# Sartor02/libMultiRobotPlanning

Measured on AMD Instinct MI355X. Metric: low_level_node_expansions_per_sec, higher is better.
Workload: dtype int32

## Files before the change

### libmultirobotplanning_amd/csrc/ll_compact.h

```cpp
#pragma once
#include <stddef.h>
#include <stdint.h>

namespace mrp {
namespace ct {

using namespace wv;

#ifndef WV_HAS_UNMASKED_GLOADS
WV_FN V gLoadU16(const uint16_t* base, V idx) { return gLoadU16m(base, idx, bsplat(true)); }
WV_FN V gLoad32(const uint32_t* base, V idx) { return gLoad32m(base, idx, bsplat(true)); }
#endif

constexpr uint32_t kRowBytes = 128;
constexpr uint32_t oCtl = 0;
constexpr uint32_t oJob = 256;
constexpr uint32_t oRes = 384;
constexpr uint32_t oOpen = 448;
constexpr uint32_t kFront = 0xFFFFFFFFu;
template <uint32_t GROUPS, uint32_t FH_BITS, uint32_t F_BITS, uint32_t L_BITS, bool LONGT = false>
struct TierCfg {
  static constexpr bool kLongT = LONGT;
  static constexpr uint32_t kGroups = GROUPS;
  static constexpr uint32_t kCap = 256u * GROUPS - 1u;
// ... 27 lines not shown
  static constexpr uint32_t pathsOff(bool bg) { return obstOff(bg) + kRowBytes; }
  static constexpr uint32_t windowBytes(bool bg) { return pathsOff(bg); }
  static_assert(kFhShift + FH_BITS == 32u, "an entry is 32 bits");
  static_assert(!LONGT || L_BITS == 6u, "h <= 62 on a 32 x 32 map");
  static constexpr uint32_t kBuildRows = LONGT ? kRows : (2u * kHeapBytes >= kRows * kRowBytes ? kRows : kRows / 2u);
  static constexpr uint32_t kStageRows = (2u * kHeapBytes + kAuxBytes) / 1024u >= 8u ? 8u : (2u * kHeapBytes + kAuxBytes) / 1024u;
  static_assert(2u * kHeapBytes >= kBuildRows * kRowBytes && kRows % kBuildRows == 0u, "room for a chunk of bitmap rows");
  static_assert(kStageRows >= 4u, "room for the goal branch's rows");
  static_assert(!LONGT || kAuxBytes >= kBitsBytes, "LONGT builds a chunk of bitmap rows in the walk queue's area");
  static_assert(oFocal % 16 == 0 && oAux % 16 == 0 && oBits % 16 == 0 && oObst % 16 == 0 && oPaths % 16 == 0, "16-byte aligned areas");
  static_assert((kHeapClamp & 1u) == 1u && 4u * (kHeapClamp + 3u) <= kHeapBytes, "clamped child pair stays inside the heap area");
  static_assert((kAuxClamp & 1u) == 1u && 4u * (kAuxClamp + 3u) <= kAuxBytes, "clamped child pair stays inside the walk queue");
  static_assert(256u * GROUPS <= kAuxIdxMask + 1u && 10u + F_BITS + L_BITS + kAuxShift <= 32u, "walk-queue entry: key above index");
  static_assert(kMaxT + 1u + 62u <= kFMax - 3u, "f = g + h (h <= 62 on a 32 x 32 map) fits its field");
};
#ifndef MRP_CT_NARROW_GROUPS
#define MRP_CT_NARROW_GROUPS 4
#endif
typedef TierCfg<MRP_CT_NARROW_GROUPS, 9, 7, 6> Narrow;
#ifndef MRP_CT_WIDE_GROUPS
#define MRP_CT_WIDE_GROUPS 12
#endif
typedef TierCfg<MRP_CT_WIDE_GROUPS, 6, 10, 6, true> Wide;
constexpr uint32_t kGroups = Narrow::kGroups, kCap = Narrow::kCap, kHeapBytes = Narrow::kHeapBytes, kAuxBytes = Narrow::kAuxBytes;
constexpr uint32_t kRows = Narrow::kRows;
constexpr uint32_t oFocal = Narrow::oFocal, oAux = Narrow::oAux, oBits = Narrow::oBits, oObst = Narrow::oObst, oPaths = Narrow::oPaths;
constexpr uint32_t kLdsBytes = oPaths;
constexpr uint32_t obstOff(bool bg) { return Narrow::obstOff(bg); }
constexpr uint32_t pathsOff(bool bg) { return Narrow::pathsOff(bg); }
constexpr uint32_t windowBytes(bool bg) { return Narrow::windowBytes(bg); }
constexpr uint32_t kBitsBytes = Narrow::kBitsBytes, kParentBytes = Narrow::kParentBytes;
constexpr uint32_t kMO = Narrow::kMO, kMF = Narrow::kMF, kEmpty = Narrow::kEmpty, kMaxT = Narrow::kMaxT;
constexpr uint32_t kHeapClamp = Narrow::kHeapClamp;
static_assert(oOpen % 16 == 0, "LDS areas are 16-byte aligned");

enum : int32_t { C_OK = 0, C_NO_SOLUTION = 1, C_CAP_EXP = 2, C_OVERFLOW = -1 };

struct CJob {
  uint32_t dimx, dimy, sx, sy, gx, gy;
  int32_t lastGoal;
  float w;
  uint32_t nVc, nEc;
  uint32_t obstWords;
  uint32_t nAgentsPad, tPad;
  uint32_t maxExp;
  uint32_t openCap, maxT;
  uint32_t taNoGoal;
  uint32_t rows;
  uint64_t vc;
  uint64_t ec;
  uint64_t obst;
  uint64_t pathsG;
  uint64_t parentTab;
  uint64_t outPath;
  uint64_t bitsG;
};
static_assert(sizeof(CJob) <= oRes - oJob && sizeof(CJob) % 4 == 0, "CJob fits its block of the window");
struct CRes {
  int32_t status, cost, fmin, nStates;
  uint32_t expanded, nodes;
};
#ifdef MRP_CT_PROF
#define MRP_CT_PROF_DECL uint32_t prof_[8] = {0, 0, 0, 0, 0, 0, 0, 0}; uint64_t profT_ = wv::clock64()
#define MRP_CT_PROF_MARK(k) do { const uint64_t n_ = wv::clock64(); prof_[k] += (uint32_t)(n_ - profT_); profT_ = n_; } while (0)
#define MRP_CT_PROF_ADD(k, v) prof_[k] += (v)
#define MRP_CT_PROF_STORE(lds) do { for (uint32_t q_ = 0; q_ < 8; ++q_) ldsStoreS(lds, oRes + 32u + 4u * q_, prof_[q_]); } while (0)
#elif defined(MRP_CT_ASM_MARKS)
#define MRP_CT_PROF_DECL do { } while (0)
#define MRP_CT_PROF_MARK(k) asm volatile("; PHASE " #k ::: "memory")
#define MRP_CT_PROF_ADD(k, v) do { } while (0)
#define MRP_CT_PROF_STORE(lds) do { } while (0)
#else
#define MRP_CT_PROF_DECL do { } while (0)
#define MRP_CT_PROF_MARK(k) do { } while (0)
#define MRP_CT_PROF_ADD(k, v) do { } while (0)
#define MRP_CT_PROF_STORE(lds) do { } while (0)
#endif
static_assert(sizeof(CRes) <= 32 && oRes + 64 <= oOpen, "CRes fits its block of the window");

#ifndef MRP_CT_COUNT
#define MRP_CT_COUNT(k, v) do { } while (0)
#endif
#ifndef MRP_CT_COUNT_SLOTS
#define MRP_CT_COUNT_SLOTS 7
#endif
#define MRP_CT_COUNTX(k, v) do { if ((k) < MRP_CT_COUNT_SLOTS) MRP_CT_COUNT(k, v); } while (0)

#define MRP_CT_JOB_U32(lds, field) ldsLoadS(lds, oJob + (uint32_t)offsetof(CJob, field))
template <class T>
WV_FN T* jobPtr(Lds lds, uint32_t off) {
  const uint64_t lo = ldsLoadS(lds, oJob + off), hi = ldsLoadS(lds, oJob + off + 4u);
  return (T*)(uintptr_t)(lo | (hi << 32));
}
#define MRP_CT_JOB_PTR(T, lds, field) jobPtr<T>(lds, (uint32_t)offsetof(CJob, field))

WV_FN uint32_t popc64(uint64_t v) { return (uint32_t)__builtin_popcountll(v); }
WV_FN uint32_t ctz64(uint64_t v) { return (uint32_t)__builtin_ctzll(v); }
WV_FN uint32_t ctz32(uint32_t v) { return (uint32_t)__builtin_ctz(v); }
WV_FN uint32_t lg2(uint32_t v) { return 31u - (uint32_t)__builtin_clz(v); }
WV_FN uint32_t lo32(uint64_t v) { return (uint32_t)v; }
WV_FN uint32_t hi32(uint64_t v) { return (uint32_t)(v >> 32); }

#ifndef WV_HAS_CTZ
WV_FN V ctz(V v) { return splat(31u) - clz(v & (splat(0u) - v)); }
#endif

#ifdef MRP_CT_PLAIN_EXPANSION
#ifndef MRP_CT_SCALAR_PUSHES
// ... 290 lines not shown
  const V dx = sel(lane == 1u, splat(0xFFFFFFFFu), sel(lane == 2u, splat(1u), sel(lane < 5u, splat(0u), splat(0x4000u))));
  const V dy = sel(lane == 3u, splat(1u), sel(lane == 4u, splat(0xFFFFFFFFu), splat(0u)));
#ifndef MRP_CT_PLAIN_EXPANSION
  const bool grid = EPS && nAgentsPad != 0u && nAgentsPad <= 16u;
#else
  const bool grid = false;
#endif
  const V agent0 = grid ? Rw.l4 : lane;
  const B in0 = agent0 < nAgentsPad, in1 = (lane + 64u) < nAgentsPad;
  const V col0 = sel(in0, agent0, splat(nAgentsPad ? nAgentsPad - 1u : 0u));
  const V col1 = sel(in1, lane + 64u, splat(nAgentsPad ? nAgentsPad - 1u : 0u));
  const V gridD = perRow(Rw, 0xFFFFFFFFu, 1u, 256u, 0xFFFFFF00u);
  const V gridSh = ((lane - 1u) & 3u) << 4;
  const V gridWait = sel(lane == 0u, splat(0xFFFFFFFFu), splat(0u));
  const uint32_t tPad = EPS ? MRP_CT_JOB_U32(lds, tPad) : 0u;
  const uint16_t* pathsG = PLDS ? nullptr : MRP_CT_JOB_PTR(const uint16_t, lds, pathsG);
  const int32_t lastGoal = (int32_t)MRP_CT_JOB_U32(lds, lastGoal);
  const float wBound = uintAsFloat(MRP_CT_JOB_U32(lds, w));
  const uint32_t maxExp = MRP_CT_JOB_U32(lds, maxExp), openCap = MRP_CT_JOB_U32(lds, openCap), maxT = MRP_CT_JOB_U32(lds, maxT);
  uint8_t* parentTab = MRP_CT_JOB_PTR(uint8_t, lds, parentTab);
  const uint32_t goalCell = gx | (gy << 5);
  int32_t bestF;
  V tops;
  {
    const uint32_t sx = MRP_CT_JOB_U32(lds, sx), sy = MRP_CT_JOB_U32(lds, sy);
    const uint32_t h0 = (sx > gx ? sx - gx : gx - sx) + (sy > gy ? sy - gy : gy - sy);
    bestF = (int32_t)h0;
    const uint32_t e0 = (kFhMax << kFhShift) | ((kFMax - h0) << kFShift) | ((C::kLongT ? 63u - h0 : 0u) << 10) | (sx | (sy << 5));
    ldsStoreS(lds, oOpen + 4u, e0);
    if (EPS) ldsStoreS(lds, oFocal + 4u, e0);
    tops = splat(e0);
  }
  sync();
  MRP_CT_PROF_MARK(0);

  for (;;) {
    if (nOpen == 0u) {
      status = C_NO_SOLUTION;
      break;
    }
#ifdef MRP_CT_LOAD_TOPS
    tops = ldsLoad32(lds, hb);
#elif defined(MRP_CT_CHECK_TOPS)
    {
      const V seen = ldsLoad32(lds, hb);
      MRP_CT_COUNTX(8, 1u);
      MRP_CT_COUNTX(9, (readlane(seen, 0) != readlane(tops, 0) || (EPS && readlane(seen, 32) != readlane(tops, 32))) ? 1u : 0u);
    }
#endif
    const uint32_t topO = readlane(tops, 0);
    uint32_t curE = EPS ? readlane(tops, 32) : topO;
    if (EPS) {
      const int32_t fTop = (int32_t)(kFMax - ((topO >> kFShift) & kFMax));
      const int32_t oldBest = bestF;
      bestF = fTop;
      if (fTop > oldBest) {
        MRP_CT_PROF_MARK(0);
        const float lo = fmulRn((float)oldBest, wBound), hi = fmulRn((float)fTop, wBound);
        bool bandEmpty = false;
#ifndef MRP_CT_FORCE_WALK
        {
          const int32_t fA = (int32_t)lo + 1, fBraw = (int32_t)hi;
          const int32_t fB = fBraw > (int32_t)kFMax - 1 ? (int32_t)kFMax - 1 : fBraw;
          bandEmpty = true;
          if (fB >= fA) {
            const V base = splat(kFMax - (uint32_t)fB), span = splat((uint32_t)(fB - fA));
            for (uint32_t g = 0; g < kGroups && g * 256u <= nOpen; ++g) {
// ... 76 lines not shown
          }
        }
        for (uint32_t b = 0; b <= 4u * npqHigh; b += 1024u) {
          const V4 none{splat(kEmpty), splat(kEmpty), splat(kEmpty), splat(kEmpty)};
          const V4 head{sel(lane == 0u, splat(kFront), splat(kEmpty)), splat(kEmpty), splat(kEmpty), splat(kEmpty)};
          ldsStore128m(lds, splat(oAux + b) + lane * 16u, b == 0u ? head : none, (lane * 16u + b) < kAuxBytes);
        }
        if (status == C_OVERFLOW) break;
        curE = ldsLoadS(lds, oFocal + 4u);
#ifndef MRP_CT_LOAD_TOPS
        tops = sel(S.isB, splat(curE), tops);
#endif
        }
        MRP_CT_PROF_MARK(1);
      }
    }
    const uint32_t cell = curE & 1023u, curFh = kFhMax - (curE >> kFhShift);
    const uint32_t t = C::kLongT ? (kFMax - ((curE >> kFShift) & kFMax)) - (63u - ((curE >> 10) & 63u)) : (curE >> 10) & kGMax;
    const uint32_t x = cell & 31u, y = cell >> 5;
    const bool isGoal = cell == goalCell && (int32_t)t > lastGoal;
    if (!isGoal) {
      if (nOpen + 5u > openCap || t > maxT || (EPS && !C::kExactFhCheck && curFh + 2u * nAgentsPad > kFhMax)) {
        status = C_OVERFLOW;
        cost = nOpen + 5u > openCap ? 1 : t > maxT ? 2 : 3;
        break;
      }
    }
    expansions += 1u;
    if (expansions > maxExp) {
      status = C_CAP_EXP;
      break;
    }
    if (isGoal) {
      status = C_OK;
      cost = (int32_t)t;
      fmin = (int32_t)(kFMax - (((EPS ? topO : curE) >> kFShift) & kFMax));
      nStates = (int32_t)t + 1;
      uint16_t* outPath = MRP_CT_JOB_PTR(uint16_t, lds, outPath);
      sync();
      uint32_t c = cell;
      const uint32_t* tab32 = (const uint32_t*)parentTab;
      constexpr int32_t kStage = BG ? (int32_t)C::kStageRows : 8;
      for (int32_t k0 = (int32_t)t; k0 >= 1; k0 -= kStage) {
        V rowW[kStage][4];
        for (int32_t r = 0; r < kStage; ++r)
          for (uint32_t q = 0; q < 4; ++q)
            rowW[r][q] = (k0 - r >= 1) ? gLoad32Coherent(tab32, splat((uint32_t)(k0 - r) * 256u + q * 64u) + lane) : splat(0u);
        for (int32_t r = 0; r < kStage; ++r)
          for (uint32_t q = 0; q < 4; ++q) ldsStore32(lds, splat(oBuild + (uint32_t)r * 1024u + q * 256u) + lane * 4u, rowW[r][q]);
        sync();
        for (int32_t r = 0; r < kStage && k0 - r >= 1; ++r) {
          const uint32_t k = (uint32_t)(k0 - r);
          gStoreU16m(outPath, splat(k), splat((c & 31u) | ((c >> 5) << 8)), lane == 0u);
          const uint32_t a = first(ldsLoadU8(lds, splat(oBuild + (uint32_t)r * 1024u + c)));
          c = a == 1u ? c + 1u : a == 2u ? c - 1u : a == 3u ? c - 32u : a == 4u ? c + 32u : c;
        }
        sync();
      }
      gStoreU16m(outPath, splat(0u), splat((c & 31u) | ((c >> 5) << 8)), lane == 0u);
      break;
    }

    MRP_CT_PROF_MARK(0);
    const uint32_t t1 = t + 1u;
    if (C::kLongT && t1 >= rowsReady) moreRows();
    const V nx = splat(x) + dx, ny = splat(y) + dy;
    const B inb = (nx < dimx) & (ny < dimy);
    const V ncell = (nx & 31u) | ((ny & 31u) << 5);
    const V wordAddr = splat(oBits + t1 * kRowBytes) + ((ny & 31u) << 2);
    const V wordIdx = splat(t1 * (kRowBytes / 4u)) + (ny & 31u);
    const V word = BG ? gLoad32(bitsG, wordIdx) : ldsLoad32(lds, wordAddr);
    V a0 = splat(0xFFFFu), b0 = splat(0xFFFFu), a1 = splat(0xFFFFu), b1 = splat(0xFFFFu);
    if (EPS && nAgentsPad) {
      const uint32_t ra = t < tPad ? t : tPad - 1u;
      const uint32_t rb = t1 < tPad ? t1 : tPad - 1u;
      if (PLDS) {
        a0 = sel(in0, ldsLoadU16(lds, splat(oPathsX + ra * nAgentsPad * 2u) + col0 * 2u), splat(0xFFFFu));
        b0 = sel(in0, ldsLoadU16(lds, splat(oPathsX + rb * nAgentsPad * 2u) + col0 * 2u), splat(0xFFFFu));
        if (nAgentsPad > 64u) {
          a1 = sel(in1, ldsLoadU16(lds, splat(oPathsX + ra * nAgentsPad * 2u) + col1 * 2u), splat(0xFFFFu));
          b1 = sel(in1, ldsLoadU16(lds, splat(oPathsX + rb * nAgentsPad * 2u) + col1 * 2u), splat(0xFFFFu));
        }
      } else {
        a0 = gLoadU16(pathsG, splat(ra * nAgentsPad) + col0);
        b0 = gLoadU16(pathsG, splat(rb * nAgentsPad) + col0);
        if (nAgentsPad > 64u) {
          a1 = gLoadU16(pathsG, splat(ra * nAgentsPad) + col1);
          b1 = gLoadU16(pathsG, splat(rb * nAgentsPad) + col1);
        }
      }
    }

// ... 420 lines not shown
```

### libmultirobotplanning_amd/csrc/ll_jobs.h

```cpp
#ifndef MRP_LL_JOBS_H
#define MRP_LL_JOBS_H

namespace mrp {

__host__ __device__ inline uint32_t ldsBytes(uint32_t pathBytes, bool bg) { return ct::windowBytes(bg) + pathBytes; }

DEVI uint32_t storeLoad(const uint16_t* p) {
#ifdef MRP_LL_STORE_ACQUIRE_FENCE
  return *p;
#else
  return __hip_atomic_load(p, __ATOMIC_RELAXED, __HIP_MEMORY_SCOPE_AGENT);
#endif
}

DEVI uint32_t hostLoad32(const uint32_t* p) { return __hip_atomic_load(p, __ATOMIC_RELAXED, __HIP_MEMORY_SCOPE_SYSTEM); }
DEVI void hostStore32(uint32_t* p, uint32_t v) { __hip_atomic_store(p, v, __ATOMIC_RELAXED, __HIP_MEMORY_SCOPE_SYSTEM); }

DEVI void stageConstraints(const uint32_t* consHost, uint32_t vcOff, uint32_t nVc, uint32_t nEc, uint32_t* consLocal,
                           const uint32_t*& vc, const uint32_t*& ec) {
  const uint32_t* src = consHost + vcOff;
  const uint32_t nWords = nVc + nEc;
  if (nWords <= kConsLocalWords) {
    for (uint32_t i = threadIdx.x; i < nWords; i += 64) consLocal[i] = hostLoad32(src + i);
    vc = consLocal;
  } else {
    __builtin_amdgcn_fence(__ATOMIC_ACQUIRE, "");
    vc = src;
  }
  ec = vc + nVc;
}

__device__ __attribute__((noinline)) bool stageConstraintSet(const DevJob* job, const uint32_t* cons, uint32_t* store, uint32_t stride,
                                                             uint32_t slots, uint32_t* consLocal) {
  const uint32_t nVc = rfl(job->n_vc), nEc = rfl(job->n_ec), dimx = rfl(job->dimx), dimy = rfl(job->dimy);
  const uint32_t baseP1 = rfl(job->pad_[0]), baseCounts = rfl(job->pad_[1]), resP1 = rfl(job->pad_[2]);
  const uint32_t* added = cons + rfl(job->vc_off);
  stride = rfl(stride); slots = rfl(slots);
  const uint32_t bVc = baseP1 ? (baseCounts & 0xFFFFu) : 0u, bEc = baseP1 ? (baseCounts >> 16) : 0u;
  const uint32_t nWords = nVc + nEc;
  if (store == nullptr || baseP1 > slots || resP1 > slots || bVc > nVc || bEc > nEc || nVc > kConsLocalWords ||
      nEc > kConsLocalWords || nWords > kConsLocalWords || nWords > stride)
    return false;
  const uint32_t aVc = nVc - bVc;
  const uint32_t cells = dimx * dimy;
  const uint32_t* base = store + (size_t)(baseP1 ? baseP1 - 1u : 0u) * stride;
  uint32_t* out = store + (size_t)(resP1 ? resP1 - 1u : 0u) * stride;
  for (uint32_t i = threadIdx.x; i < nWords; i += 64) {
    uint32_t w;
    if (i < nVc) {
// ... 197 lines not shown
  }
  return true;
}

template <bool EPS, bool BG, int TIERS>
DEVI bool compactAttempt(const LaunchParams& P, const DevJob& J, uint8_t* smem, uint8_t* arenaSlot, const Ctx& c, DevResult& res,
                         uint16_t* outPath, SState& s, int& rc) {
  typedef typename std::conditional<TIERS == kTiersHeavy, ct::Wide, ct::Narrow>::type Geo;
  uint32_t geoRows = Geo::kRows;
  if (TIERS == kTiersHeavy) {
    const uint64_t room = slot::nodeBytes(P.arena_nodes) / (1024u + ct::kRowBytes);
    geoRows = (uint32_t)(room < P.arena_rows ? room : P.arena_rows) & ~63u;
  }
  const bool compactOk = !(TIERS == kTiersAll && (J.ctx_flags & kCtxHeavy) != 0) && P.lds_nodes != 0 && c.dimx <= 32u &&
                         c.dimy <= 32u && c.nAgentsPad <= 128u && c.nEc <= 64u && geoRows >= 64u &&
                         compactFits<Geo>(P.arena_nodes, geoRows, BG);
  bool done = false;
  if (compactOk) {
    ct::CJob cj = baseCJob<Geo>(P, J, arenaSlot, outPath, geoRows);
    cj.obstWords = c.wpr;
    cj.sx = c.sx; cj.sy = c.sy; cj.gx = c.gx; cj.gy = c.gy;
    cj.lastGoal = c.lastGoal;
    cj.nVc = c.nVc; cj.nEc = c.nEc;
    cj.nAgentsPad = EPS ? c.nAgentsPad : 0u; cj.tPad = c.tPad;
    cj.rows = geoRows;
    if (TIERS == kTiersHeavy) {
      cj.openCap = Geo::kCap;
      cj.maxT = Geo::kMaxT < geoRows - 2u ? Geo::kMaxT : geoRows - 2u;
    }
    cj.vc = (uint64_t)c.vc; cj.ec = (uint64_t)c.ec;
    cj.pathsG = (uint64_t)c.paths;
    putCJob(smem, cj);
    const bool tableInLds = !EPS || c.nAgentsPad == 0u || c.pathsLds != nullptr;
#ifndef MRP_LL_TRACE
    const uint64_t tl0 = __builtin_amdgcn_s_memrealtime();
#endif
    int32_t crc;
    if constexpr (TIERS == kTiersHeavy)
      crc = ct::compactSearch<EPS, false, BG, ct::Wide>((wv::Lds)smem);
    else
      crc = tableInLds ? ct::compactSearch<EPS, true, BG>((wv::Lds)smem) : ct::compactSearch<EPS, false, BG>((wv::Lds)smem);
    const ct::CRes cr = getCRes(smem);
#ifndef MRP_LL_TRACE
    res.prof[TIERS == kTiersHeavy ? 2 : 0] = (uint32_t)(__builtin_amdgcn_s_memrealtime() - tl0);
    res.prof[TIERS == kTiersHeavy ? 3 : 1] = cr.expanded;
#endif
#ifdef MRP_CT_PROF
    {
      auto r32 = (__attribute__((address_space(3))) const uint32_t*)((wv::Lds)smem + ct::oRes + 32u);
      for (uint32_t q = 0; q < 8; ++q) res.prof[q] = rfl(r32[q]);
    }
#endif
    if (crc != ct::C_OVERFLOW) {
      rc = crc;
      res.cost = cr.cost; res.fmin = cr.fmin; res.n_states = cr.nStates;
      s.expansions = cr.expanded; s.nNodes = cr.nodes;
      done = true;
      if (TIERS == kTiersHeavy) res.tier = 2;
    } else {
#ifndef MRP_LL_TRACE
      res.prof[6] = cr.expanded;
      res.prof[7] = 1;
#endif
    }
  }
  return done;
}

template <bool EPS, bool BG, int TIERS>
DEVI int arenaAttempt(const LaunchParams& P, uint8_t* smem, uint8_t* arenaSlot, const Ctx& c, DevResult& res, uint16_t* outPath,
                      SState& s) {
  typedef typename std::conditional<TIERS == kTiersHeavy, ct::Wide, ct::Narrow>::type Geo;
  int rc;
  const Mem<TierHbm> g = cutArena(P, arenaSlot);
  Mem<TierHyb> gh = viewAs<TierHyb>(g);
  {
    const uint32_t area = Geo::windowBytes(BG) - ct::oOpen;
#ifdef MRP_LL_TOPS_EQUAL
    const uint32_t perO = (area / 3u) & ~15u, perF = perO, perA = perO;
#else
    const uint32_t perO = (area / 2u) & ~15u, perF = (area * 5u / 16u) & ~15u, perA = (area - perO - perF) & ~15u;
#endif
    auto tops = [&](uint32_t per) {
      uint32_t n = per >= 32u ? ((per - 8u) / 8u) : 0u;
      if (n > 4095u) n = 4095u;
      n = n ? ((n - 1u) | 1u) : 0u;
      return P.lds_nodes == 0 ? 0u : n;
    };
    auto l8 = (__attribute__((address_space(3))) uint8_t*)smem + ct::oOpen;
    gh.open = HybPtr{(__attribute__((address_space(3))) uint64_t*)(l8 + 8), (uint64_t*)g.open, tops(perO)};
    gh.focal = HybPtr{(__attribute__((address_space(3))) uint64_t*)(l8 + perO + 8), (uint64_t*)g.focal, tops(perF)};
    gh.aux = HybPtr{(__attribute__((address_space(3))) uint64_t*)(l8 + perO + perF + 8), (uint64_t*)g.aux, tops(perA)};
  }
  const bool xyEntries = P.arena_nodes <= 65536u;
  Mem<TierHybXy> ghx = viewAs<TierHybXy>(gh);
  res.tier = 1;
  __syncthreads();
  if (xyEntries)
    initSearch<TierHybXy, EPS>(ghx, s, c);
  else
    initSearch<TierHyb, EPS>(gh, s, c);
  __syncthreads();
#ifndef MRP_LL_TRACE
  const uint64_t th0 = __builtin_amdgcn_s_memrealtime();
#endif
  if (xyEntries)
    rc = runSearch<TierHybXy, EPS>(ghx, s, c, res, outPath);
  else
    rc = runSearch<TierHyb, EPS>(gh, s, c, res, outPath);
#ifndef MRP_LL_TRACE
  if (TIERS != kTiersHeavy) {
    res.prof[2] = (uint32_t)(__builtin_amdgcn_s_memrealtime() - th0);
    res.prof[3] = (uint32_t)s.expansions;
  }
#endif
  return rc;
}

template <bool EPS, bool BG, int TIERS>
DEVI bool runJob(const LaunchParams& P, const DevJob& J, uint8_t* smem, uint8_t* arenaSlot, DevResult& res,
                 uint16_t* outPath) {
  typedef typename std::conditional<TIERS == kTiersHeavy, ct::Wide, ct::Narrow>::type Geo;
  if (TIERS == kTiersFront && frontHandsOver(P, J)) return true;
  Ctx c;
  fillCtx(c, J, P.maps, P.debug);
  uint32_t* consLocal = slot::consCopy(arenaSlot, P.arena_scratch_off, P.out_stride);
  if ((J.pad_[0] | J.pad_[2]) != 0u) {
    c.vc = consLocal;
    c.ec = consLocal + c.nVc;
  } else {
    stageConstraints(P.cons, J.vc_off, c.nVc, c.nEc, consLocal, c.vc, c.ec);
  }
  if (!stageFocalTable<TIERS>(P, J, smem + Geo::windowBytes(BG), slot::pathsCopy(arenaSlot, P.arena_scratch_off, P.out_stride), c)) {
    res.status = ST_BAD; res.expanded = 0; res.nodes_created = 0;
    return false;
  }
  __syncthreads();
  SState s;
  int rc = ST_BAD;
  res.tier = 0;
  if (!compactAttempt<EPS, BG, TIERS>(P, J, smem, arenaSlot, c, res, outPath, s, rc)) {
    if constexpr (TIERS == kTiersFront)
      return true;
    else
      rc = arenaAttempt<EPS, BG, TIERS>(P, smem, arenaSlot, c, res, outPath, s);
  }
  if (rc == RUN_MIGRATE_NODES) rc = ST_CAP_NODES;
  if (rc == RUN_MIGRATE_ROWS) rc = ST_CAP_HORIZON;
  res.status = rc;
  res.expanded = s.expansions;
  res.nodes_created = s.nNodes;
  return false;
}

template <class SidFn>
DEVI void publishPath(const LaunchParams& P, const uint16_t* outPath, uint32_t len, uint32_t* hostDst, SidFn sidOf) {
  const uint32_t lane = threadIdx.x;
  const uint32_t* src = (const uint32_t*)outPath;
  for (uint32_t i = lane; i < (len + 1u) / 2u; i += 64) hostStore32(hostDst + i, src[i]);
  const uint32_t sid = sidOf();
  if (sid < P.path_store_slots && len < P.path_store_stride) {
    uint16_t* slot = P.path_store + (size_t)sid * P.path_store_stride;
    for (uint32_t i = lane; i < len; i += 64) __hip_atomic_store(slot + 1 + i, outPath[i], __ATOMIC_RELAXED, __HIP_MEMORY_SCOPE_AGENT);
    __hip_atomic_store(slot, (uint16_t)len, __ATOMIC_RELAXED, __HIP_MEMORY_SCOPE_AGENT);
  }
}

template <bool HOSTLOADS>
DEVI void beginJob(const DevJob* jobSrc, DevJob& jobS, DevResult& res, uint32_t tier) {
  const uint32_t lane = threadIdx.x;
  const uint32_t* src = (const uint32_t*)jobSrc;
  __syncthreads();
  if (lane < sizeof(DevJob) / 4) ((uint32_t*)&jobS)[lane] = HOSTLOADS ? hostLoad32(src + lane) : src[lane];
  __syncthreads();
  res.status = ST_BAD; res.cost = 0; res.fmin = 0; res.n_states = 0; res.expanded = 0; res.nodes_created = 0;
  res.tier = tier;
  for (int q = 0; q < 8; ++q) res.prof[q] = 0;
}
DEVI void endJob(const DevResult& res, DevResult& resS, DevResult* resDst) {
  __syncthreads();
  resS = res;
  __syncthreads();
  if (threadIdx.x < sizeof(DevResult) / 4) hostStore32((uint32_t*)resDst + threadIdx.x, ((const uint32_t*)&resS)[threadIdx.x]);
}

DEVI void runChain(const LaunchParams& P, const DevJob& J, uint8_t* smem, uint8_t* arenaSlot, DevResult& res,
                   uint16_t* outPath, uint16_t* hostOut) {
  constexpr bool BG = true;
  const uint32_t lane = threadIdx.x;
  const uint32_t n = J.n_ctx, first = J.t_pad, npad = J.n_agents_pad;
  const uint32_t end = J.reserved > first && J.reserved < n ? J.reserved : n;
  res.tier = 0; res.n_states = 0; res.expanded = 0;
  if (P.lds_nodes == 0 || J.dimx > 32u || J.dimy > 32u || n > kChainMaxAgents || first >= n || npad < n || npad > 128u ||
      (npad & 1u) || kChainRows * npad * 2u > (P.lds_paths_bytes != 0u ? P.lds_paths_bytes : P.arena_paths_bytes) ||
      !compactFits<ct::Narrow>(P.arena_nodes, 0, BG) ||
      (uint64_t)n * kChainEntryWords * 2u + (uint64_t)n * 64u > (uint64_t)P.out_host_stride) {
    res.status = ST_BAD;
    return;
  }
  const uint32_t* who = P.cons + J.vc_off;
  const uint32_t* ids = who + n;
  const bool tabInLds = P.lds_paths_bytes != 0u;
  uint16_t* table = (uint16_t*)(tabInLds ? smem + ldsBytes(0, BG) : slot::pathsCopy(arenaSlot, P.arena_scratch_off, P.out_stride));
  for (uint32_t i = lane; i < kChainRows * npad / 2u; i += 64) ((uint32_t*)table)[i] = 0xFFFFFFFFu;
  __syncthreads();
  for (uint32_t a = 0; a < first; ++a) {
    const uint32_t id = rfl(hostLoad32(ids + a));
    if (id >= P.path_store_slots) continue;
    const uint16_t* slot = P.path_store + (size_t)id * P.path_store_stride;
    uint32_t len = rfl(storeLoad(slot));
    if (len > P.path_store_stride - 1) len = P.path_store_stride - 1;
    if (len == 0) continue;
    table[lane * npad + a] = (uint16_t)storeLoad(slot + 1 + (lane < len ? lane : len - 1));
  }
  __syncthreads();
  int64_t budget = J.max_expansions;
  uint32_t* hostW = (uint32_t*)hostOut;
  uint32_t pathOff = n * kChainEntryWords;
  uint32_t done = 0, maxLen = 0;
  bool allOk = true;
  int64_t total = 0;
  for (uint32_t a = first; a < end; ++a) {
    asm volatile("" : "+s"(hostW), "+s"(outPath));
    const uint32_t sg = rfl(hostLoad32(who + a));
    ct::CJob cj = baseCJob(P, J, arenaSlot, outPath);
    cj.sx = sg & 0xFFu; cj.sy = (sg >> 8) & 0xFFu; cj.gx = (sg >> 16) & 0xFFu; cj.gy = sg >> 24;
    cj.lastGoal = -1;
    cj.nVc = 0; cj.nEc = 0;
    cj.nAgentsPad = npad; cj.tPad = kChainRows;
    cj.maxExp = clampMaxExp(budget);
    cj.vc = 0; cj.ec = 0;
    cj.pathsG = tabInLds ? 0ull : (uint64_t)table;
    __syncthreads();
    putCJob(smem, cj);
#ifndef MRP_LL_TRACE
    const uint64_t tl0 = __builtin_amdgcn_s_memrealtime();
#endif
    const int32_t crc = tabInLds ? ct::compactSearch<true, true, BG>((wv::Lds)smem) : ct::compactSearch<true, false, BG>((wv::Lds)smem);
    const ct::CRes cr = getCRes(smem);
    const int32_t cost = cr.cost, fmin = cr.fmin, nStates = cr.nStates;
    const uint32_t expanded = cr.expanded;
#ifndef MRP_LL_TRACE
    res.prof[0] += (uint32_t)(__builtin_amdgcn_s_memrealtime() - tl0);
    res.prof[1] += expanded;
#endif
    if (crc == ct::C_OVERFLOW) {
#ifndef MRP_LL_TRACE
      res.prof[6] += expanded;
      res.prof[7] += 1;
#endif
      allOk = false;
      break;
    }
    {
      uint32_t v = 0;
      v = lane == 0 ? (uint32_t)crc : lane == 1 ? (uint32_t)cost : lane == 2 ? (uint32_t)fmin
          : lane == 3 ? (crc == ct::C_OK ? (uint32_t)nStates : 0u) : lane == 4 ? expanded : lane == 5 ? pathOff : 0u;
      if (lane < kChainEntryWords) hostStore32(hostW + (size_t)done * kChainEntryWords + lane, v);
    }
    done += 1;
    total += expanded;
    if (crc != ct::C_OK) {
      allOk = false;
      break;
    }
    const uint32_t len = (uint32_t)nStates;
    maxLen = len > maxLen ? len : maxLen;
    {
      publishPath(P, outPath, len, hostW + pathOff, [&] { return rfl(hostLoad32(ids + a)); });
      pathOff += (len + 1u) / 2u;
      uint32_t rowLen = npad;
      asm volatile("" : "+s"(rowLen));
      table[lane * rowLen + a] = outPath[lane < len ? lane : len - 1];
    }
    if (budget >= 0) budget = budget > (int64_t)expanded ? budget - (int64_t)expanded : 0;
  }
  __syncthreads();
  res.status = ST_OK;
  res.n_states = (int32_t)done;
  res.expanded = total;
  res.cost = -1;
  res.fmin = -1;
  if (first == 0 && end == n && done == n && allOk && maxLen >= 1u && maxLen <= kChainRows) {
    const uint32_t T = maxLen - 1u;
    uint32_t cnt = 0, key = 0x7FFFFFFFu;
    auto pairsOf = [&](const uint16_t* tab, uint32_t rowC, uint32_t rowN, uint32_t t, bool inT) {
      uint32_t bestV = 0xFFFFu, bestE = 0xFFFFu;
      for (uint32_t i = 0; i + 1u < n; ++i) {
        const uint32_t ci = tab[rowC + i], ni = tab[rowN + i];
        for (uint32_t j = i + 1u; j < n; ++j) {
          const uint32_t cj = tab[rowC + j], nj = tab[rowN + j];
          const bool v = inT && ci == cj, e = inT && ci == nj && ni == cj;
          cnt += (v ? 1u : 0u) + (e ? 1u : 0u);
          if (v && bestV == 0xFFFFu) bestV = (i << 8) | j;
          if (e && bestE == 0xFFFFu) bestE = (i << 8) | j;
        }
      }
      const uint32_t k = bestV != 0xFFFFu ? (t << 24) | bestV : bestE != 0xFFFFu ? (t << 24) | (1u << 16) | bestE : 0x7FFFFFFFu;
      key = k < key ? k : key;
    };
    if (tabInLds) {
      pairsOf(table, lane * npad, (lane + 1u < kChainRows ? lane + 1u : kChainRows - 1u) * npad, lane, lane < T);
    } else {
      uint16_t* stage = (uint16_t*)(smem + ct::oOpen);
      static_assert(2u * ct::kHeapBytes >= 32u * kChainMaxAgents * 2u, "room for 32 rows of the widest table");
      const uint32_t rowsFit = 2u * ct::kHeapBytes / (npad * 2u) < kChainRows ? 2u * ct::kHeapBytes / (npad * 2u) : kChainRows;
      for (uint32_t r0 = 0; r0 < T; r0 += rowsFit - 1u) {
        const uint32_t nRows = kChainRows - r0 < rowsFit ? kChainRows - r0 : rowsFit;
        __syncthreads();
        for (uint32_t i = lane; i < nRows * npad / 2u; i += 64) ((uint32_t*)stage)[i] = ((const uint32_t*)table)[r0 * npad / 2u + i];
        __syncthreads();
        const bool inT = lane + 1u < nRows && r0 + lane < T;
        const uint32_t row = inT ? lane : 0u;
        pairsOf(stage, row * npad, (row + 1u) * npad, r0 + lane, inT);
      }
    }
#pragma unroll
    for (uint32_t off = 32; off >= 1; off >>= 1) {
      cnt += (uint32_t)__shfl_xor((int)cnt, (int)off, 64);
      const uint32_t other = (uint32_t)__shfl_xor((int)key, (int)off, 64);
      key = other < key ? other : key;
    }
    res.cost = (int32_t)rfl(cnt);
    res.fmin = rfl(key) == 0x7FFFFFFFu ? -1 : (int32_t)rfl(key);
  }
}

}

#endif
```

### libmultirobotplanning_amd/csrc/ll_kernel.hip

```cpp
#include <hip/hip_runtime.h>
#include <stdint.h>

#include <mutex>
#include <type_traits>

#include "ll_device.h"
#include "ll_slot.h"
#include "ll_launch.h"
#include "wave_dev.h"
#include "ll_compact.h"

#include "ll_arena_heap.h"
#include "ll_arena_search.h"
#include "ll_jobs.h"
#include "ll_ta.h"
#include "ll_ta_root.h"
#include "ll_ta_eps_root.h"
#include "ll_sipp.h"
#include "ll_node_scan.h"

namespace mrp {

constexpr uint32_t kScanJobOff = ct::oCtl + sizeof(DevJob) + sizeof(DevResult), kScanOutOff = kScanJobOff + sizeof(ns::NsJob);
constexpr uint32_t kScanBaseOff = ct::oCtl + sizeof(DevJob);
// ... 63 lines not shown
                     uint8_t* arenaSlot, DevJob& jobS, DevResult& resS) {
  static_assert(TIERS == kTiersAll || KIND == 1, "front / heavy workgroups exist for the A*-epsilon sessions");
  const DevJob& J = jobS;
  DevResult res;
  beginJob<true>(jobSrc, jobS, res, 0);
  PROF_T0();
#ifndef MRP_LL_TRACE
  const uint64_t tj0 = __builtin_amdgcn_s_memrealtime();
#endif
  uint16_t* outPath = slot::outPath(arenaSlot, P.arena_scratch_off, P.out_stride);
  uint32_t algo = rfl(J.algo);
  bool handOver = false;
  if ((rfl(J.pad_[0]) | rfl(J.pad_[2])) != 0u && !(TIERS == kTiersFront && frontHandsOver(P, J))) {
    if (algo > 1u || (rfl(J.ctx_flags) & kCtxChain) ||
        !stageConstraintSet(&jobS, P.cons, P.cons_store, P.cons_store_stride, P.cons_store_slots,
                            slot::consCopy(arenaSlot, P.arena_scratch_off, P.out_stride)))
      algo = 0xFFFFFFFFu;
  }
  if constexpr (KIND == 0) {
    if (algo == 1)
      runJob<true, false, kTiersAll>(P, J, smem, arenaSlot, res, outPath);
    else if (algo == 3)
      runJobTA(P, J, smem, arenaSlot, res, outPath);
    else if (algo == 4) {
      const uint64_t th0 = __builtin_amdgcn_s_memrealtime();
      runJobTaEps<false>(&jobS, &resS, arenaSlot, P.maps, P.cons, P.paths, P.arena_scratch_off, P.out_stride, P.arena_nodes,
                  P.arena_rows, P.arena_row_words, P.arena_paths_bytes, P.path_store, P.path_store_stride, P.path_store_slots);
      __syncthreads();
      res.status = rfli(resS.status); res.cost = rfli(resS.cost); res.fmin = rfli(resS.fmin);
      res.n_states = rfli(resS.n_states);
      res.expanded = (int64_t)rfl64((uint64_t)resS.expanded);
      res.nodes_created = rfl(resS.nodes_created);
      res.tier = rfl(resS.tier);
      res.prof[2] = (uint32_t)(__builtin_amdgcn_s_memrealtime() - th0);
      res.prof[3] = (uint32_t)res.expanded;
    } else if (algo == 0)
      runJob<false, false, kTiersAll>(P, J, smem, arenaSlot, res, outPath);
  } else if constexpr (KIND == 1) {
    if (algo == 1) {
      if (rfl(J.ctx_flags) & kCtxChain) {
        if constexpr (TIERS != kTiersHeavy) runChain(P, J, smem, arenaSlot, res, outPath, pathDst);
      } else {
        handOver = runJob<true, true, TIERS>(P, J, smem, arenaSlot, res, outPath);
      }
    }
  } else {
    if (algo == 0) runJob<false, false, kTiersAll>(P, J, smem, arenaSlot, res, outPath);
    if (algo == 3) runJobTA(P, J, smem, arenaSlot, res, outPath);
  }
  if (TIERS == kTiersFront && handOver) return true;
  if constexpr (KIND != 2) {
    if (rfl(J.ctx_flags) & kCtxScan)
      scanNode<KIND == 1, TIERS>(P, J, smem, arenaSlot, (int32_t)rfl((uint32_t)res.status), rfl((uint32_t)res.n_states), outPath, pathDst);
  }
  PROF_ADD(res, 5);
#if !defined(MRP_LL_TRACE) && !defined(MRP_CT_PROF)
  res.prof[4] = (uint32_t)(__builtin_amdgcn_s_memrealtime() - tj0);
  res.prof[5] = 1;
#endif
  DBG(P, 2, res.status + 100);
  endJob(res, resS, resDst);
  if (res.status == ST_OK && !(KIND == 1 && (rfl(J.ctx_flags) & kCtxChain)))
    publishPath(P, outPath, (uint32_t)res.n_states, (uint32_t*)pathDst, [&] { return rfl(J.store_out_id); });
  return false;
}

static_assert(sizeof(DevJob) + sizeof(DevResult) <= ct::oJob, "control block of the window");
#define MRP_LL_WINDOW_BLOCKS(smem, jobS, resS)                                                        \
  if ((uint32_t)(uintptr_t)(__attribute__((address_space(3))) uint8_t*)smem != 0u) __builtin_trap(); \
  DevJob& jobS = *(DevJob*)(smem + ct::oCtl);                                                         \
  DevResult& resS = *(DevResult*)(smem + ct::oCtl + sizeof(DevJob))
#define MRP_LL_WINDOW_KERNEL(NAME, ...)                                                  \
  extern "C" __global__ void __launch_bounds__(64) NAME(LaunchParams Parg) {             \
    extern __shared__ __attribute__((aligned(16))) uint8_t smem[];                       \
    MRP_LL_WINDOW_BLOCKS(smem, jobS, resS);                                              \
    const LaunchParams& P = Parg;                                                        \
    __VA_ARGS__(P, smem, jobS, resS);                                                    \
  }
template <int KIND>
DEVI void batchLoop(const LaunchParams& P, uint8_t* smem, DevJob& jobS, DevResult& resS) {
  const uint32_t lane = threadIdx.x;
  uint8_t* arenaSlot = P.arena + (size_t)blockIdx.x * P.arena_stride;
  DBG(P, 0, 1);
  for (;;) {
    uint32_t j = atomicAdd(P.queue_head, lane == 0 ? 1u : 0u);
    j = rfl(j) - P.queue_base;
    DBG(P, 1, j + 1);
    if (j >= P.n_jobs) break;
    processJob<KIND>(P, P.jobs + j, P.results + j, P.out_paths + (size_t)j * P.out_host_stride, smem, arenaSlot, jobS, resS);
// ... 317 lines not shown
```

Before: 1.487 billion.

## Keep goal path in lanes and stage chain pairs to skip host reads

For non-long-time tiers, the goal backtrack now collects the path in a wave register, one lane per state, instead of storing one global u16 per step. That removes the per-step global stores and the syncs around each staged walk, and the path is written once to global and to an LDS copy. The chain runner stages the who/id pairs into scratch up front rather than doing per-agent host loads. It then publishes paths and fills the table from the LDS copy instead of re-reading global outPath. It also adds optional profiling macros, and the LDS copy overlaps the aux area, which is a correctness risk.

Result: faster. 1.505 billion, median of 5 (+1.3%).

```diff
diff --git a/libmultirobotplanning_amd/csrc/ll_compact.h b/libmultirobotplanning_amd/csrc/ll_compact.h
--- a/libmultirobotplanning_amd/csrc/ll_compact.h
+++ b/libmultirobotplanning_amd/csrc/ll_compact.h
@@ -83,6 +83,7 @@
 constexpr uint32_t kBitsBytes = Narrow::kBitsBytes, kParentBytes = Narrow::kParentBytes;
 constexpr uint32_t kMO = Narrow::kMO, kMF = Narrow::kMF, kEmpty = Narrow::kEmpty, kMaxT = Narrow::kMaxT;
 constexpr uint32_t kHeapClamp = Narrow::kHeapClamp;
+constexpr uint32_t kPathCopyStates = 64, oPathCopy = Narrow::oAux + Narrow::kAuxBytes - 4u * kPathCopyStates;
 static_assert(oOpen % 16 == 0, "LDS areas are 16-byte aligned");
 
 enum : int32_t { C_OK = 0, C_NO_SOLUTION = 1, C_CAP_EXP = 2, C_OVERFLOW = -1 };
@@ -112,19 +113,26 @@
   uint32_t expanded, nodes;
 };
 #ifdef MRP_CT_PROF
+#define MRP_CT_PROF_FIXED ((MRP_CT_PROF + 0) == 2)
 #define MRP_CT_PROF_DECL uint32_t prof_[8] = {0, 0, 0, 0, 0, 0, 0, 0}; uint64_t profT_ = wv::clock64()
 #define MRP_CT_PROF_MARK(k) do { const uint64_t n_ = wv::clock64(); prof_[k] += (uint32_t)(n_ - profT_); profT_ = n_; } while (0)
-#define MRP_CT_PROF_ADD(k, v) prof_[k] += (v)
+#define MRP_CT_PROF_ADD(k, v) do { if (!MRP_CT_PROF_FIXED) prof_[k] += (v); } while (0)
+#define MRP_CT_PROF_MARK_SETUP() MRP_CT_PROF_MARK(MRP_CT_PROF_FIXED ? 6 : 0)
+#define MRP_CT_PROF_MARK_GOAL(k) do { if (MRP_CT_PROF_FIXED) MRP_CT_PROF_MARK(k); } while (0)
 #define MRP_CT_PROF_STORE(lds) do { for (uint32_t q_ = 0; q_ < 8; ++q_) ldsStoreS(lds, oRes + 32u + 4u * q_, prof_[q_]); } while (0)
 #elif defined(MRP_CT_ASM_MARKS)
 #define MRP_CT_PROF_DECL do { } while (0)
 #define MRP_CT_PROF_MARK(k) asm volatile("; PHASE " #k ::: "memory")
 #define MRP_CT_PROF_ADD(k, v) do { } while (0)
+#define MRP_CT_PROF_MARK_SETUP() MRP_CT_PROF_MARK(0)
+#define MRP_CT_PROF_MARK_GOAL(k) do { } while (0)
 #define MRP_CT_PROF_STORE(lds) do { } while (0)
 #else
 #define MRP_CT_PROF_DECL do { } while (0)
 #define MRP_CT_PROF_MARK(k) do { } while (0)
 #define MRP_CT_PROF_ADD(k, v) do { } while (0)
+#define MRP_CT_PROF_MARK_SETUP() do { } while (0)
+#define MRP_CT_PROF_MARK_GOAL(k) do { } while (0)
 #define MRP_CT_PROF_STORE(lds) do { } while (0)
 #endif
 static_assert(sizeof(CRes) <= 32 && oRes + 64 <= oOpen, "CRes fits its block of the window");
@@ -481,7 +489,7 @@
     tops = splat(e0);
   }
   sync();
-  MRP_CT_PROF_MARK(0);
+  MRP_CT_PROF_MARK_SETUP();
 
   for (;;) {
     if (nOpen == 0u) {
@@ -624,6 +632,7 @@
       break;
     }
     if (isGoal) {
+      MRP_CT_PROF_MARK_GOAL(0);
       status = C_OK;
       cost = (int32_t)t;
       fmin = (int32_t)(kFMax - (((EPS ? topO : curE) >> kFShift) & kFMax));
@@ -633,23 +642,65 @@
       uint32_t c = cell;
       const uint32_t* tab32 = (const uint32_t*)parentTab;
       constexpr int32_t kStage = BG ? (int32_t)C::kStageRows : 8;
-      for (int32_t k0 = (int32_t)t; k0 >= 1; k0 -= kStage) {
-        V rowW[kStage][4];
+      static_assert(!BG || C::kLongT || oOpen + (uint32_t)kStage * 1024u <= C::obstOff(true), "the staged rows end in front of the obstacle row");
+      constexpr bool kPathCopy = !C::kLongT;
+#ifndef MRP_CT_PLAIN_EXPANSION
+      constexpr bool kPathInLanes = kPathCopy;
+#else
+      constexpr bool kPathInLanes = false;
+#endif
+      static_assert(!kPathCopy || (C::kGMax < kPathCopyStates && oPathCopy >= C::oAux && oPathCopy + 4u * kPathCopyStates <= C::oAux + C::kAuxBytes),
+                    "a lane per state; the copy lies in the walk queue's area");
+      static_assert(!kPathCopy || !BG || oOpen + (uint32_t)kStage * 1024u <= oPathCopy, "the staged rows end in front of the copy");
+      V pathV = splat(0u);
+      if (kPathCopy && !kPathInLanes) ldsStore32(lds, splat(oPathCopy) + lane * 4u, splat(0u));
+      auto keep = [&](uint32_t k, uint32_t cc) {
+        const uint32_t xy = (cc & 31u) | ((cc >> 5) << 8);
+        if (kPathInLanes) {
+          pathV = writelane(pathV, xy, k);
+        } else {
+          gStoreU16m(outPath, splat(k), splat(xy), lane == 0u);
+          if (kPathCopy) ldsStoreS(lds, oPathCopy + 4u * k, xy);
+        }
+      };
+      V rowW[kStage][4];
+      auto request = [&](int32_t k0) {
         for (int32_t r = 0; r < kStage; ++r)
           for (uint32_t q = 0; q < 4; ++q)
             rowW[r][q] = (k0 - r >= 1) ? gLoad32Coherent(tab32, splat((uint32_t)(k0 - r) * 256u + q * 64u) + lane) : splat(0u);
+      };
+      auto stage = [&]() {
         for (int32_t r = 0; r < kStage; ++r)
           for (uint32_t q = 0; q < 4; ++q) ldsStore32(lds, splat(oBuild + (uint32_t)r * 1024u + q * 256u) + lane * 4u, rowW[r][q]);
-        sync();
+      };
+      auto walk = [&](int32_t k0) {
         for (int32_t r = 0; r < kStage && k0 - r >= 1; ++r) {
-          const uint32_t k = (uint32_t)(k0 - r);
-          gStoreU16m(outPath, splat(k), splat((c & 31u) | ((c >> 5) << 8)), lane == 0u);
+          keep((uint32_t)(k0 - r), c);
           const uint32_t a = first(ldsLoadU8(lds, splat(oBuild + (uint32_t)r * 1024u + c)));
           c = a == 1u ? c + 1u : a == 2u ? c - 1u : a == 3u ? c - 32u : a == 4u ? c + 32u : c;
         }
-        sync();
-      }
-      gStoreU16m(outPath, splat(0u), splat((c & 31u) | ((c >> 5) << 8)), lane == 0u);
+      };
+      if (kPathInLanes) {
+        for (int32_t k0 = (int32_t)t; k0 >= 1; k0 -= kStage) {
+          request(k0);
+          stage();
+          walk(k0);
+        }
+      } else {
+        for (int32_t k0 = (int32_t)t; k0 >= 1; k0 -= kStage) {
+          request(k0);
+          stage();
+          sync();
+          walk(k0);
+          sync();
+        }
+      }
+      keep(0u, c);
+      if (kPathInLanes) {
+        gStoreU16m(outPath, lane, pathV, lane <= t);
+        ldsStore32(lds, splat(oPathCopy) + lane * 4u, pathV);
+      }
+      MRP_CT_PROF_MARK_GOAL(7);
       break;
     }
 
diff --git a/libmultirobotplanning_amd/csrc/ll_jobs.h b/libmultirobotplanning_amd/csrc/ll_jobs.h
--- a/libmultirobotplanning_amd/csrc/ll_jobs.h
+++ b/libmultirobotplanning_amd/csrc/ll_jobs.h
@@ -15,6 +15,17 @@
 
 DEVI uint32_t hostLoad32(const uint32_t* p) { return __hip_atomic_load(p, __ATOMIC_RELAXED, __HIP_MEMORY_SCOPE_SYSTEM); }
 DEVI void hostStore32(uint32_t* p, uint32_t v) { __hip_atomic_store(p, v, __ATOMIC_RELAXED, __HIP_MEMORY_SCOPE_SYSTEM); }
+
+#if !defined(MRP_LL_TRACE) && !defined(MRP_CHAIN_PROF)
+#define MRP_LL_TIER_STATS 1
+#endif
+#ifdef MRP_CHAIN_PROF
+#define MRP_CHAIN_PROF_T0() uint64_t chainT_ = __builtin_amdgcn_s_memrealtime()
+#define MRP_CHAIN_PROF_MARK(res, k) do { const uint64_t n_ = __builtin_amdgcn_s_memrealtime(); (res).prof[k] += (uint32_t)(n_ - chainT_); chainT_ = n_; } while (0)
+#else
+#define MRP_CHAIN_PROF_T0() do { } while (0)
+#define MRP_CHAIN_PROF_MARK(res, k) do { } while (0)
+#endif
 
 DEVI void stageConstraints(const uint32_t* consHost, uint32_t vcOff, uint32_t nVc, uint32_t nEc, uint32_t* consLocal,
                            const uint32_t*& vc, const uint32_t*& ec) {
@@ -278,7 +289,7 @@
     cj.pathsG = (uint64_t)c.paths;
     putCJob(smem, cj);
     const bool tableInLds = !EPS || c.nAgentsPad == 0u || c.pathsLds != nullptr;
-#ifndef MRP_LL_TRACE
+#ifdef MRP_LL_TIER_STATS
     const uint64_t tl0 = __builtin_amdgcn_s_memrealtime();
 #endif
     int32_t crc;
@@ -287,7 +298,7 @@
     else
       crc = tableInLds ? ct::compactSearch<EPS, true, BG>((wv::Lds)smem) : ct::compactSearch<EPS, false, BG>((wv::Lds)smem);
     const ct::CRes cr = getCRes(smem);
-#ifndef MRP_LL_TRACE
+#ifdef MRP_LL_TIER_STATS
     res.prof[TIERS == kTiersHeavy ? 2 : 0] = (uint32_t)(__builtin_amdgcn_s_memrealtime() - tl0);
     res.prof[TIERS == kTiersHeavy ? 3 : 1] = cr.expanded;
 #endif
@@ -304,7 +315,7 @@
       done = true;
       if (TIERS == kTiersHeavy) res.tier = 2;
     } else {
-#ifndef MRP_LL_TRACE
+#ifdef MRP_LL_TIER_STATS
       res.prof[6] = cr.expanded;
       res.prof[7] = 1;
 #endif
@@ -347,14 +358,14 @@
   else
     initSearch<TierHyb, EPS>(gh, s, c);
   __syncthreads();
-#ifndef MRP_LL_TRACE
+#ifdef MRP_LL_TIER_STATS
   const uint64_t th0 = __builtin_amdgcn_s_memrealtime();
 #endif
   if (xyEntries)
     rc = runSearch<TierHybXy, EPS>(ghx, s, c, res, outPath);
   else
     rc = runSearch<TierHyb, EPS>(gh, s, c, res, outPath);
-#ifndef MRP_LL_TRACE
+#ifdef MRP_LL_TIER_STATS
   if (TIERS != kTiersHeavy) {
     res.prof[2] = (uint32_t)(__builtin_amdgcn_s_memrealtime() - th0);
     res.prof[3] = (uint32_t)s.expansions;
@@ -375,7 +386,9 @@
     c.vc = consLocal;
     c.ec = consLocal + c.nVc;
   } else {
-    stageConstraints(P.cons, J.vc_off, c.nVc, c.nEc, consLocal, c.vc, c.ec);
+    const uint32_t* consHost = P.cons;
+    if constexpr (TIERS == kTiersFront) asm volatile("" : "+s"(consHost), "+s"(consLocal));
+    stageConstraints(consHost, J.vc_off, c.nVc, c.nEc, consLocal, c.vc, c.ec);
   }
   if (!stageFocalTable<TIERS>(P, J, smem + Geo::windowBytes(BG), slot::pathsCopy(arenaSlot, P.arena_scratch_off, P.out_stride), c)) {
     res.status = ST_BAD; res.expanded = 0; res.nodes_created = 0;
@@ -434,6 +447,7 @@
                    uint16_t* outPath, uint16_t* hostOut) {
   constexpr bool BG = true;
   const uint32_t lane = threadIdx.x;
+  MRP_CHAIN_PROF_T0();
   const uint32_t n = J.n_ctx, first = J.t_pad, npad = J.n_agents_pad;
   const uint32_t end = J.reserved > first && J.reserved < n ? J.reserved : n;
   res.tier = 0; res.n_states = 0; res.expanded = 0;
@@ -444,14 +458,24 @@
     res.status = ST_BAD;
     return;
   }
-  const uint32_t* who = P.cons + J.vc_off;
-  const uint32_t* ids = who + n;
+  const uint32_t* who = P.cons + rfl(J.vc_off);
+  const uint32_t* ids = who + rfl(n);
   const bool tabInLds = P.lds_paths_bytes != 0u;
   uint16_t* table = (uint16_t*)(tabInLds ? smem + ldsBytes(0, BG) : slot::pathsCopy(arenaSlot, P.arena_scratch_off, P.out_stride));
   for (uint32_t i = lane; i < kChainRows * npad / 2u; i += 64) ((uint32_t*)table)[i] = 0xFFFFFFFFu;
+  uint32_t* staged = slot::consCopy(arenaSlot, P.arena_scratch_off, P.out_stride);
+  static_assert(2u * kChainMaxAgents <= kConsLocalWords, "room for the chain's pairs");
+  asm volatile("" : "+s"(who), "+s"(ids), "+s"(staged));
+  for (uint32_t a0 = 0; a0 < n; a0 += 64) {
+    if (a0 + lane < n) {
+      const uint32_t w = hostLoad32(who + a0 + lane), id = hostLoad32(ids + a0 + lane);
+      staged[2u * (a0 + lane)] = w;
+      staged[2u * (a0 + lane) + 1u] = id;
+    }
+  }
   __syncthreads();
   for (uint32_t a = 0; a < first; ++a) {
-    const uint32_t id = rfl(hostLoad32(ids + a));
+    const uint32_t id = __builtin_amdgcn_readlane(staged[2u * a + (lane & 1u)], 1);
     if (id >= P.path_store_slots) continue;
     const uint16_t* slot = P.path_store + (size_t)id * P.path_store_stride;
     uint32_t len = rfl(storeLoad(slot));
@@ -466,9 +490,11 @@
   uint32_t done = 0, maxLen = 0;
   bool allOk = true;
   int64_t total = 0;
+  MRP_CHAIN_PROF_MARK(res, 0);
   for (uint32_t a = first; a < end; ++a) {
-    asm volatile("" : "+s"(hostW), "+s"(outPath));
-    const uint32_t sg = rfl(hostLoad32(who + a));
+    asm volatile("" : "+s"(hostW), "+s"(outPath), "+s"(staged));
+    const uint32_t pair = staged[2u * a + (lane & 1u)];
+    const uint32_t sg = __builtin_amdgcn_readlane(pair, 0), sid = __builtin_amdgcn_readlane(pair, 1);
     ct::CJob cj = baseCJob(P, J, arenaSlot, outPath);
     cj.sx = sg & 0xFFu; cj.sy = (sg >> 8) & 0xFFu; cj.gx = (sg >> 16) & 0xFFu; cj.gy = sg >> 24;
     cj.lastGoal = -1;
@@ -479,23 +505,34 @@
     cj.pathsG = tabInLds ? 0ull : (uint64_t)table;
     __syncthreads();
     putCJob(smem, cj);
-#ifndef MRP_LL_TRACE
+    MRP_CHAIN_PROF_MARK(res, 1);
+#ifdef MRP_LL_TIER_STATS
     const uint64_t tl0 = __builtin_amdgcn_s_memrealtime();
 #endif
     const int32_t crc = tabInLds ? ct::compactSearch<true, true, BG>((wv::Lds)smem) : ct::compactSearch<true, false, BG>((wv::Lds)smem);
     const ct::CRes cr = getCRes(smem);
     const int32_t cost = cr.cost, fmin = cr.fmin, nStates = cr.nStates;
     const uint32_t expanded = cr.expanded;
-#ifndef MRP_LL_TRACE
+    MRP_CHAIN_PROF_MARK(res, 2);
+#ifdef MRP_CHAIN_PROF
+    res.prof[5] += 1;
+#endif
+#ifdef MRP_CT_PROF
+    {
+      auto r32 = (__attribute__((address_space(3))) const uint32_t*)((wv::Lds)smem + ct::oRes + 32u);
+      for (uint32_t q = 0; q < 8; ++q) res.prof[q] += rfl(r32[q]);
+    }
+#elif defined(MRP_LL_TIER_STATS)
     res.prof[0] += (uint32_t)(__builtin_amdgcn_s_memrealtime() - tl0);
     res.prof[1] += expanded;
 #endif
     if (crc == ct::C_OVERFLOW) {
-#ifndef MRP_LL_TRACE
+#if defined(MRP_LL_TIER_STATS) && !defined(MRP_CT_PROF)
       res.prof[6] += expanded;
       res.prof[7] += 1;
 #endif
       allOk = false;
+      MRP_CHAIN_PROF_MARK(res, 3);
       break;
     }
     {
@@ -508,18 +545,28 @@
     total += expanded;
     if (crc != ct::C_OK) {
       allOk = false;
+      MRP_CHAIN_PROF_MARK(res, 3);
       break;
     }
     const uint32_t len = (uint32_t)nStates;
     maxLen = len > maxLen ? len : maxLen;
     {
-      publishPath(P, outPath, len, hostW + pathOff, [&] { return rfl(hostLoad32(ids + a)); });
+      auto pc = (__attribute__((address_space(3))) const uint32_t*)((wv::Lds)smem + ct::oPathCopy);
+      const uint32_t mine = pc[lane];
+      if (lane < (len + 1u) / 2u) hostStore32(hostW + pathOff + lane, pc[2u * lane] | (pc[2u * lane + 1u] << 16));
       pathOff += (len + 1u) / 2u;
+      if (sid < P.path_store_slots && len < P.path_store_stride) {
+        uint16_t* slot = P.path_store + (size_t)sid * P.path_store_stride;
+        if (lane < len) __hip_atomic_store(slot + 1 + lane, (uint16_t)mine, __ATOMIC_RELAXED, __HIP_MEMORY_SCOPE_AGENT);
+        __hip_atomic_store(slot, (uint16_t)len, __ATOMIC_RELAXED, __HIP_MEMORY_SCOPE_AGENT);
+      }
       uint32_t rowLen = npad;
       asm volatile("" : "+s"(rowLen));
-      table[lane * rowLen + a] = outPath[lane < len ? lane : len - 1];
+      const uint32_t last = __builtin_amdgcn_readlane(mine, len - 1u);
+      table[lane * rowLen + a] = (uint16_t)(lane < len ? mine : last);
     }
     if (budget >= 0) budget = budget > (int64_t)expanded ? budget - (int64_t)expanded : 0;
+    MRP_CHAIN_PROF_MARK(res, 3);
   }
   __syncthreads();
   res.status = ST_OK;
@@ -570,8 +617,9 @@
     res.cost = (int32_t)rfl(cnt);
     res.fmin = rfl(key) == 0x7FFFFFFFu ? -1 : (int32_t)rfl(key);
   }
-}
-
-}
-
-#endif
+  MRP_CHAIN_PROF_MARK(res, 4);
+}
+
+}
+
+#endif
diff --git a/libmultirobotplanning_amd/csrc/ll_kernel.hip b/libmultirobotplanning_amd/csrc/ll_kernel.hip
--- a/libmultirobotplanning_amd/csrc/ll_kernel.hip
+++ b/libmultirobotplanning_amd/csrc/ll_kernel.hip
@@ -119,8 +119,12 @@
       res.expanded = (int64_t)rfl64((uint64_t)resS.expanded);
       res.nodes_created = rfl(resS.nodes_created);
       res.tier = rfl(resS.tier);
+#ifndef MRP_CHAIN_PROF
       res.prof[2] = (uint32_t)(__builtin_amdgcn_s_memrealtime() - th0);
       res.prof[3] = (uint32_t)res.expanded;
+#else
+      (void)th0;
+#endif
     } else if (algo == 0)
       runJob<false, false, kTiersAll>(P, J, smem, arenaSlot, res, outPath);
   } else if constexpr (KIND == 1) {
@@ -141,7 +145,12 @@
       scanNode<KIND == 1, TIERS>(P, J, smem, arenaSlot, (int32_t)rfl((uint32_t)res.status), rfl((uint32_t)res.n_states), outPath, pathDst);
   }
   PROF_ADD(res, 5);
-#if !defined(MRP_LL_TRACE) && !defined(MRP_CT_PROF)
+#ifdef MRP_CHAIN_PROF
+  if (KIND == 1 && algo == 1 && (rfl(J.ctx_flags) & kCtxChain)) {
+    res.prof[6] = (uint32_t)(__builtin_amdgcn_s_memrealtime() - tj0);
+    res.prof[7] = 1;
+  }
+#elif !defined(MRP_LL_TRACE) && !defined(MRP_CT_PROF)
   res.prof[4] = (uint32_t)(__builtin_amdgcn_s_memrealtime() - tj0);
   res.prof[5] = 1;
 #endif
```
